# huangjh-pub/di-fusion

Measured on AMD Instinct MI355X. Metric: frames/s integrate+decode+mesh, 640x480 synthetic stream, higher is better.
Workload: dtype f32

## Files before the change

### di_fusion_amd/_lib.py

```python
from __future__ import annotations

import ctypes
import os
from ctypes import POINTER, Structure, c_float, c_int32, c_int64, c_uint8, c_void_p
from pathlib import Path

PKG = Path(__file__).resolve().parent
LIB_PATH = Path(os.environ["DIF_LIB"]) if os.environ.get("DIF_LIB") else PKG / "libdifusion.so"

C_N_OCCUPIED, C_OVERFLOW, C_ALLOC_NEW, C_M, C_C, C_ITEMS, C_K, C_B, C_VH, C_T, C_QUERY_M, C_N_KEPT, C_CACHE_T, C_CACHE_KEPT, C_EXPORT_N, C_WORK, C_CACHE_DEAD, C_CACHE_LIVE, C_OPT_ROWS, C_OPT_VOXELS, C_HALO_L, C_HALO_R, C_HALO_TICKET, C_DEFERRED = range(24)
C_STAMP = 31
SYNC_FUSED, SYNC_FRONT_DONE, SYNC_WORDS = 0, 32, 64
FC_COUNT = 32
C_COUNT = 32
PROF_NAMES = ["encode", "decode_lattice", "decode_points", "mc_count", "mc_emit", "halo_export", "halo_merge"]
PROF_COUNT = 8
LATENT_DIM = 29

ERRORS = {-1: "DIF_EINVAL (bad argument)", -2: "DIF_ELAUNCH (HIP launch/runtime failure)", -3: "DIF_ENOSPACE (workspace too small)"}


class DifMap(Structure):
    _fields_ = [("nx", c_int32), ("ny", c_int32), ("nz", c_int32),
                ("bound_min", c_float * 3), ("voxel_size", c_float),
# ... 65 lines not shown
    "dif_compute_normal_weight": (c_int32, [c_void_p, c_void_p, c_int32, c_int32, c_void_p]),
    "dif_filter_depth": (c_int32, [c_void_p, c_void_p, c_int32, c_int32, c_void_p]),
    "dif_depth_frontend": (c_int32, [c_void_p, c_int32, c_int32, c_float, c_float, c_float, c_float, c_int32, c_void_p, c_void_p, c_void_p,
                                     c_void_p, c_void_p, c_void_p]),
    "dif_point_box_filter": (c_int32, [c_void_p, c_void_p, c_int64, c_float, c_void_p, c_void_p, c_void_p, c_void_p, c_int64, c_void_p,
                                       c_void_p, c_void_p, c_void_p]),
    "dif_cloud_workspace_bytes": (c_int64, [c_int64]),
    "dif_knn": (c_int32, [c_void_p, c_int64, c_int32, c_int32, c_float, c_void_p, c_void_p, c_void_p, c_int64, c_void_p]),
    "dif_remove_radius_outlier": (c_int32, [c_void_p, c_int64, c_int32, c_int32, c_float, c_void_p, c_void_p, c_int64, c_void_p]),
    "dif_estimate_normals": (c_int32, [c_void_p, c_int64, c_int32, c_int32, c_float, POINTER(c_float), c_void_p, c_void_p, c_int64,
                                       c_void_p]),
    "dif_groupby_sum": (c_int32, [c_void_p, c_void_p, c_int64, c_int32, c_void_p, c_void_p, c_int64, c_void_p]),
    "dif_integrate_workspace_bytes": (c_int64, [c_int64]),
    "dif_integrate": (c_int32, [POINTER(DifMap), POINTER(DifWeights), c_void_p, c_void_p, c_int64, c_void_p, c_void_p,
                                c_int64, c_void_p]),
    "dif_integrate_frame": (c_int32, [POINTER(DifMap), POINTER(DifWeights), c_void_p, c_int32, c_int32, c_float, c_float, c_float, c_float,
                                      c_void_p, c_void_p, c_void_p, c_void_p, c_int64, c_void_p]),
    "dif_optimize_workspace_bytes": (c_int64, [c_int64, c_int64]),
    "dif_optimize_latents": (c_int32, [POINTER(DifMap), POINTER(DifWeights), c_void_p, c_void_p, c_int64, c_void_p, c_void_p, c_int32, c_float,
                                       c_float, c_void_p, c_void_p, c_int64, c_void_p]),
    "dif_extract": (c_int32, [POINTER(DifMap), POINTER(DifWeights), POINTER(DifExtractBuffers), c_int32, c_int32, c_float,
                              c_int32, c_int32, c_void_p]),
    "dif_integrate_frames": (c_int32, [POINTER(DifStreamFrame), c_int32, POINTER(DifWeights), c_int32, c_int32, c_float, c_float, c_float, c_float,
                                       c_void_p]),
    "dif_extract_streams": (c_int32, [POINTER(DifStreamFrame), c_int32, POINTER(DifWeights), c_int32, c_float, c_int32, c_void_p]),
    "dif_export_pending": (c_int32, [POINTER(DifMap), c_void_p]),
    "dif_mesh_cache_export": (c_int32, [POINTER(DifExtractBuffers), c_int64, c_int64, c_void_p, c_void_p, c_void_p, c_void_p]),
    "dif_mesh_cache_export_dma": (c_int32, [POINTER(DifExtractBuffers), c_int64, c_int64, c_void_p, c_void_p, c_void_p, c_void_p]),
    "dif_mesh_cache_compact": (c_int32, [POINTER(DifMap), POINTER(DifExtractBuffers), c_void_p, c_void_p, c_void_p, c_int64, c_void_p, c_void_p]),
    "dif_mesh_cache_reindex": (c_int32, [POINTER(DifMap), POINTER(DifExtractBuffers), c_int64, c_void_p]),
    "dif_marching_cubes": (c_int32, [c_void_p, c_int32, c_int32, c_int32, c_void_p, c_int64, c_void_p, c_int64, c_void_p,
                                     c_void_p, c_int32, c_float, c_int64, c_void_p, c_void_p, c_void_p, c_void_p,
                                     c_void_p, c_void_p, c_void_p, c_void_p]),
    "dif_decode_rows": (c_int32, [POINTER(DifWeights), c_void_p, c_int64, c_void_p, c_void_p, c_void_p]),
    "dif_encode_rows": (c_int32, [POINTER(DifWeights), c_void_p, c_int64, c_void_p, c_void_p]),
    "dif_query_sdf": (c_int32, [POINTER(DifMap), POINTER(DifWeights), c_void_p, c_int64, c_void_p, c_void_p, c_void_p,
                                c_void_p, c_void_p, c_void_p, c_void_p]),
    "dif_query_select": (c_int32, [POINTER(DifMap), c_void_p, c_int64, c_void_p, c_void_p, c_void_p, c_void_p, c_int32, c_void_p]),
    "dif_query_decode": (c_int32, [POINTER(DifMap), POINTER(DifWeights), c_void_p, c_int64, c_void_p, c_void_p, c_void_p, c_void_p, c_void_p]),
    "dif_query_grad_scatter": (c_int32, [c_void_p, c_void_p, c_void_p, c_int64, c_void_p, c_void_p]),
    "dif_query_grad_gather": (c_int32, [c_void_p, c_void_p, c_void_p, c_int64, c_void_p, c_void_p]),
    "dif_export_records": (c_int32, [POINTER(DifMap), c_void_p, c_int64, c_int32, c_int32, c_int32, c_void_p, c_void_p]),
    "dif_merge_records": (c_int32, [POINTER(DifMap), c_void_p, c_int64, c_int32, c_void_p, c_void_p]),
    "dif_export_halo": (c_int32, [POINTER(DifMap), c_void_p, c_int64, c_int32, c_int32, c_void_p, c_void_p]),
    "dif_merge_halo": (c_int32, [POINTER(DifMap), c_void_p, c_int64, c_void_p, c_void_p]),
    "dif_export_halo_delta": (c_int32, [POINTER(DifMap), c_void_p, c_void_p, c_int64, c_void_p, c_void_p]),
    "dif_halo_lists_reset": (c_int32, [POINTER(DifMap), c_void_p, c_void_p, c_void_p, c_void_p]),
    "dif_merge_halo2": (c_int32, [POINTER(DifMap), c_void_p, c_int64, c_void_p, c_int64, c_void_p, c_void_p, c_void_p]),
    "dif_profile_enable": (c_int32, [c_int32]),
    "dif_profile_read": (c_int32, [POINTER(ctypes.c_double), POINTER(c_int64), c_int32]),
    "dif_profile_dump": (c_int64, [POINTER(c_int32), POINTER(c_float), c_int64, c_int32]),
    "dif_read_counters": (c_int32, [POINTER(DifMap), POINTER(c_int32), c_void_p]),
    "dif_test_mc_grid_cap": (c_int32, [c_int32]),
    "dif_test_sdma_mode": (c_int32, [c_int32]),
    "dif_sdma_info": (c_int32, [POINTER(c_int32)]),
    "dif_test_handoff": (c_int32, [c_int32, c_int32, c_int32, c_int32, POINTER(c_int64)]),
    "dif_queues_independent": (c_int32, [c_void_p, c_void_p]),
    "dif_mesh_cache_export_sdma": (c_int32, [POINTER(DifExtractBuffers), c_int64, c_int64, c_void_p, c_void_p, c_void_p]),
    "dif_sdf_hg_workspace_bytes": (c_int64, [c_int64]),
    "dif_sdf_hg": (c_int32, [POINTER(DifMap), POINTER(DifWeights), c_void_p, c_int64, POINTER(DifSdfHg), c_void_p, c_int64, c_void_p, c_void_p,
                             c_int64, c_void_p]),
    "dif_gradient_xy": (c_int32, [c_void_p, c_int32, c_int32, c_void_p, c_void_p]),
    "dif_photo_pyramid": (c_int32, [c_void_p, c_void_p, c_int32, c_int32, POINTER(DifPhotoPyramid), c_void_p]),
    "dif_rgb_odometry": (c_int32, [c_void_p, c_void_p, c_void_p, c_void_p, c_void_p, c_int32, c_int32, POINTER(DifRgbHg), c_void_p, c_void_p,
                                   c_void_p]),
    "dif_rgb_hg_workspace_bytes": (c_int64, []),
    "dif_rgb_hg": (c_int32, [c_void_p, c_void_p, c_void_p, c_void_p, c_void_p, c_int32, c_int32, POINTER(DifRgbHg), c_void_p, c_int64, c_void_p,
                             c_void_p, c_int64, c_void_p]),
}

_lib = None


def load() -> ctypes.CDLL:
    global _lib
    if _lib is None:
        import torch
        if not LIB_PATH.exists():
            raise RuntimeError(f"{LIB_PATH} is missing: build it with `python -c 'import __graft_entry__ as g; g.build()'` "
                               "(hipcc, gfx950). di_fusion_amd has no CPU fallback.")
        if not os.environ.get("DIF_LIB"):
            from . import _build
            have, want = _build.lib_build_id(), _build.source_hash()
            if have != want:
                try:
                    _build.build(force=True, verbose=False, shared=True)
                except Exception as e:
                    raise RuntimeError(f"{LIB_PATH} was built from other sources (build id {have}, tree {want}) and rebuilding it failed: {e!r}")
        lib = ctypes.CDLL(str(LIB_PATH))
        for name, (res, args) in SIGNATURES.items():
            fn = getattr(lib, name)
            fn.restype = res
            fn.argtypes = args
        _lib = lib
    return _lib


def spin_until(words, index: int, value: int, what: str, timeout_s: float = 30.0):
    import time
    if words[index] == value:
        return
    t0 = time.perf_counter()
    n = 0
    while words[index] != value:
        n += 1
        if (n & 0x3FFF) == 0 and time.perf_counter() - t0 > timeout_s:
# ... 29 lines not shown
```

### di_fusion_amd/csrc/difusion.hip

```cpp
#include <cstdlib>
#include <cstdio>
#include <cstring>
#include <mutex>
#include <atomic>
#include <chrono>
#include <vector>
#include <hip/hip_runtime.h>
#include <hsa/hsa.h>
#include <hsa/hsa_ext_amd.h>
#include <dlfcn.h>

#include "common.hip.h"
#include "mlp.hip.h"
#include "mc_tables.inc"

using namespace dif;

namespace {

constexpr int L = DIF_LATENT_DIM;

__device__ __constant__ int c_mc_edge_table[256];
__device__ __constant__ unsigned long long c_mc_tri_packed[256];
bool g_tables_uploaded[64] = {};
// ... 859 lines not shown
    a.max_triangles = buf->cache_capacity; a.new_limit = buf->max_triangles; a.base_ptr = C + DIF_C_CACHE_KEPT;
    a.triangles = buf->cache_tri; a.tri_id = buf->cache_id; a.tri_std = buf->cache_std; a.tri_alive = buf->cache_alive;
    a.scale = scale_vertices ? 1 : 0; a.vs = map->voxel_size; a.bx = map->bound_min[0]; a.by = map->bound_min[1]; a.bz = map->bound_min[2];
    a.log_counters = C;
    a.grid_tot = map->grid_tot;
    if (2 * (e.r + 1) * (e.r + 1) * (e.r + 1) <= e.R3) {
        a.corner_cache = reinterpret_cast<float*>(buf->refine_list);
        a.corner_stride = e.R3;
    }
    return a;
}

static bool defer_export_of(const dif_map_t* map, const dif_extract_buffers_t* buf) {
    return buf->defer_export && map->pending_export && buf->out_tri && buf->out_id && buf->out_std;
}

static void mc_onepass_args(McArgs& a, const dif_map_t* map, const dif_extract_buffers_t* buf, bool defer) {
    a.tri_start = map->tri_start; a.tri_n = map->tri_n; a.tri_count = buf->tri_count; a.tri_offset = nullptr;
    if (!defer && buf->out_tri && buf->out_id && buf->out_std) {
        a.out_tri = buf->out_tri; a.out_id = buf->out_id; a.out_std = buf->out_std; a.out_capacity = buf->out_capacity;
    }
}

static FinishArgs finish_args_of(const dif_map_t* map, const dif_extract_buffers_t* buf, bool fused_scan, bool onepass, bool exported, bool defer) {
    int32_t* const super_sum = buf->chunk_sum ? buf->chunk_sum + (buf->max_voxels + 255) / 256 : nullptr;
    const bool ov = overlapped(map);
    return FinishArgs{buf->occ_slot, map->vbm, map->counters, buf->max_triangles, buf->cache_capacity, buf->cache_tri, buf->cache_id, buf->cache_std,
                      ExtractOut{buf->counters_out, buf->out_tri, buf->out_id, buf->out_std, buf->out_capacity, (exported || defer) ? 1 : 0,
                                 defer ? (dif_pending_export_t*)map->pending_export : nullptr, buf->stamp, defer ? buf->export_notify : nullptr},
                      (fused_scan && !onepass) ? buf->chunk_sum : nullptr, super_sum, map->dirty_tot, (int)((map->capacity + DIF_BLOCK - 1) / DIF_BLOCK),
                      onepass ? buf->mc_status : nullptr, onepass ? buf->mc_status + (buf->max_voxels + 3) / 4 : nullptr,
                      ov ? map->frame_counters : nullptr};
}

static int voxel_decode_attributes() {
    static bool attr_set[64] = {};
    int dev = 0; (void)hipGetDevice(&dev);
    if (dev < 64 && !attr_set[dev]) {
        const int fp32_bytes = (int)(((size_t)((DEC_LDS_FLOATS + 3) & ~3) + 4 * VD_WAVE_LDS_FLOATS) * 4);
        const int x6_bytes = (int)((size_t)X6_LDS_BYTES + 4 * VD_WAVE_LDS_FLOATS * 4);
        if (hipFuncSetAttribute((const void*)k_decode_voxels<false>, hipFuncAttributeMaxDynamicSharedMemorySize, fp32_bytes) != hipSuccess) return DIF_ELAUNCH;
        if (hipFuncSetAttribute((const void*)k_decode_voxels<true>, hipFuncAttributeMaxDynamicSharedMemorySize, x6_bytes) != hipSuccess) return DIF_ELAUNCH;
        if (hipFuncSetAttribute((const void*)k_decode_refine_x6, hipFuncAttributeMaxDynamicSharedMemorySize, (int)X6_LDS_BYTES) != hipSuccess) return DIF_ELAUNCH;
        if (hipFuncSetAttribute((const void*)k_decode_voxels_batch<true>, hipFuncAttributeMaxDynamicSharedMemorySize, x6_bytes) != hipSuccess) return DIF_ELAUNCH;
        if (hipFuncSetAttribute((const void*)k_decode_refine_x6_batch, hipFuncAttributeMaxDynamicSharedMemorySize, (int)X6_LDS_BYTES) != hipSuccess) return DIF_ELAUNCH;
        attr_set[dev] = true;
    }
    return DIF_OK;
}

static std::atomic<int> g_mc_grid_cap{0};
int dif_test_mc_grid_cap(int32_t n) { return g_mc_grid_cap.exchange(n > 0 ? n : 0); }

static int mc_onepass_setup(const McArgs& a, size_t& lds_bytes, int& grid1, int64_t max_voxels) {
    if (upload_tables() != DIF_OK) return DIF_ELAUNCH;
    const int r = a.R / 2, nc = (r + 1) * (r + 1) * (r + 1);
    lds_bytes = (size_t)(DIF_BLOCK / 64) * MC_ONEPASS_WAVE_LDS_FLOATS(nc) * sizeof(float);
    if (lds_bytes > 128 * 1024) return DIF_EINVAL;
    static bool attr_set1[64] = {};
    int dev = 0; (void)hipGetDevice(&dev);
    if (dev < 64 && !attr_set1[dev]) {
        if (hipFuncSetAttribute((const void*)k_marching_cubes_onepass<0>, hipFuncAttributeMaxDynamicSharedMemorySize, 128 * 1024) != hipSuccess) return DIF_ELAUNCH;
        if (hipFuncSetAttribute((const void*)k_marching_cubes_onepass<4>, hipFuncAttributeMaxDynamicSharedMemorySize, 128 * 1024) != hipSuccess) return DIF_ELAUNCH;
        if (hipFuncSetAttribute((const void*)k_marching_cubes_onepass_batch<0>, hipFuncAttributeMaxDynamicSharedMemorySize, 128 * 1024) != hipSuccess) return DIF_ELAUNCH;
        if (hipFuncSetAttribute((const void*)k_marching_cubes_onepass_batch<4>, hipFuncAttributeMaxDynamicSharedMemorySize, 128 * 1024) != hipSuccess) return DIF_ELAUNCH;
        attr_set1[dev] = true;
    }
    const int64_t need = (max_voxels + 3) / 4;
    int per_cu = (int)((160 * 1024) / (lds_bytes + 1024));
    per_cu = per_cu < 1 ? 1 : per_cu > MC_WAVES_PER_SIMD ? MC_WAVES_PER_SIMD : per_cu;
    grid1 = per_cu * num_cus();
    if (need < grid1) grid1 = (int)(need < 1 ? 1 : need);
    { const int n = g_mc_grid_cap.load(std::memory_order_relaxed); if (n > 0 && n < grid1) grid1 = n; }
    return DIF_OK;
}

static int extract_mesh_part(const dif_map_t* map, const dif_extract_buffers_t* buf, const ExtractGeo& e, float max_std, int32_t no_cache,
                             int32_t scale_vertices, hipStream_t s);

static int extract_impl(const dif_map_t* map, const dif_weights_t* w, const dif_extract_buffers_t* buf, int32_t resolution, int32_t fast,
                        float max_std, int32_t no_cache, int32_t scale_vertices, void* stream_) {
    if (!map || !w || !buf || resolution < 1 || resolution > 8 || buf->max_voxels <= 0) return DIF_EINVAL;
    const int* n_slots = map->counters + DIF_C_N_OCCUPIED;
    if (!map->grid_tot) return DIF_EINVAL;
    const GridMarks bits = grid_marks_of(map);
    if (buf->cache_capacity <= 0 || buf->cache_capacity >= ((int64_t)1 << 31) || !buf->cache_tri || !buf->cache_id || !buf->cache_std || !buf->cache_alive)
        return DIF_EINVAL;
    if (!map->tri_start || !map->tri_n) return DIF_EINVAL;
    hipStream_t s = (hipStream_t)stream_;
    const int64_t grid = (int64_t)map->nx * map->ny * map->nz;
    Geo g = geo_of(map);
    int* C = map->counters;
    const bool ov = overlapped(map);
    if (ov && (!overlap_ok(map) || no_cache || defer_export_of(map, buf) || s != (hipStream_t)map->fuse_stream)) return DIF_EINVAL;
    const ExtractGeo e = extract_geo(resolution);
    const int r = e.r, R = e.R, l = e.l, R3 = e.R3;
    if (buf->max_voxels * (int64_t)R3 >= ((int64_t)1 << 31)) return DIF_EINVAL;
    const double sample_a = e.sample_a, sample_b = e.sample_b;

    {
        const DirtySet ds = dirty_set_of(map, buf, no_cache);
        const bool tiled = ds.tiled;
        if (tiled) {
            hipLaunchKernelGGL(k_mark_halo_dirty, dim3(grid_for(map->capacity, DIF_BLOCK, 256)), dim3(DIF_BLOCK), 0, s, g, map->ignore_count_th, map->dirty,
                               (const int64_t*)map->latent_vecs_pos, (const int64_t*)map->indexer, (const float*)map->voxel_obs_count, bits,
                               n_slots, ds.own_lin_lo, ds.own_lin_hi);
            DIF_CHECK_LAUNCH();
        }
        {
            DirtyFunctor f{ds};
            if (map->dirty_tot && !no_cache && !tiled && map->capacity > 4096 && map->capacity % DIF_BLOCK == 0) {
                hipLaunchKernelGGL(k_dirty_scan, dim3((int)(map->capacity / DIF_BLOCK)), dim3(DIF_BLOCK), 0, s, ds, n_slots, (const int*)map->dirty_tot,
                                   ov ? map->sync_words + DIF_SYNC_FUSED : nullptr, (int)map->frame_seq);
                DIF_CHECK_LAUNCH();
            } else if (ov) {
                return DIF_EINVAL;
            } else if (map->dirty_tot && !no_cache && !tiled) {
                if (launch_counted_scan_bounded(f, n_slots, map->capacity, map->dirty_tot, s) != DIF_OK) return DIF_ELAUNCH;
            } else if (launch_scan(f, n_slots, 0, map->capacity, buf->block_tmp, s) != DIF_OK) return DIF_ELAUNCH;
        }
    }
    {
        OccFunctor f{map->grid_bits, map->indexer, buf->occ_slot, map->vbm, C, buf->max_voxels};
        if (launch_counted_scan(f, (int)((grid + 31) / 32), map->grid_tot, s) != DIF_OK) return DIF_ELAUNCH;
    }
    int rc;
    if (fast && l * l * l <= VD_MAX_L3 && R * R <= VD_MAX_R2) {
        if (!w->dec_packed || w->dec_packed_floats != DEC_FLOATS) return DIF_EINVAL;
        const bool fold = w->dec_fold_packed && w->dec_fold_packed_floats == DECF_FLOATS && buf->fold_table;
        const VoxelDecodeArgs V = voxel_decode_args_of(map, w, buf, e, fold);
        const bool x6 = fold && w->dec_x6_packed && w->dec_x6_packed_bytes == X6_BYTES;
        const size_t lds_bytes = x6 ? (size_t)X6_LDS_BYTES + 4 * VD_WAVE_LDS_FLOATS * 4
                                    : ((size_t)((DEC_LDS_FLOATS + 3) & ~3) + 4 * VD_WAVE_LDS_FLOATS) * 4;
        if (voxel_decode_attributes() != DIF_OK) return DIF_ELAUNCH;
        int64_t blocks = (buf->max_voxels + 3) / 4;
        if (blocks > num_cus()) blocks = num_cus();
        {
            ProfScope prof(DIF_PROF_DECODE_LATTICE, s);
            if (x6) hipLaunchKernelGGL(k_decode_voxels<true>, dim3((int)blocks), dim3(512), lds_bytes, s, V, (const float*)w->dec_x6_packed);
            else hipLaunchKernelGGL(k_decode_voxels<false>, dim3((int)blocks), dim3(512), lds_bytes, s, V, w->dec_packed);
        }
        DIF_CHECK_LAUNCH();
        const DecodeArgs Rf = refine_args_of(map, buf, e, fold);
        if (x6) {
            int64_t rblocks = (buf->max_voxels * (int64_t)(R3 / 32) + 7) / 8;
            if (rblocks < 1) rblocks = 1;
            if (rblocks > num_cus()) rblocks = num_cus();
            ProfScope prof(DIF_PROF_DECODE_POINTS, s);
            hipLaunchKernelGGL(k_decode_refine_x6, dim3((int)rblocks), dim3(512), (size_t)X6_LDS_BYTES, s, Rf, (const float*)w->dec_x6_packed);
            DIF_CHECK_LAUNCH();
            rc = DIF_OK;
        } else {
            rc = launch_decode(Rf, w, buf->max_voxels * (int64_t)(R3 / 32), s);
        }
        if (rc != DIF_OK) return rc;
    } else if (fast) {
        DecodeArgs A = {};
        A.mode = 0; A.n_ptr = C + DIF_C_B; A.occ_slot = buf->occ_slot; A.latent = map->latent_vecs;
        A.lat.res = l; A.lat.a = (float)sample_a;
        A.lat.vsize = (l > 1) ? (float)((sample_b - sample_a) / (l - 1)) : 0.0f;
        A.out_sdf = buf->low_sdf; A.out_std = buf->low_std; A.sign = 1.0f;
        rc = launch_decode(A, w, buf->max_voxels * ((l * l * l + 31) / 32), s);
        if (rc != DIF_OK) return rc;
        hipLaunchKernelGGL(k_upsample_mark, dim3(grid_for(buf->max_voxels * (int64_t)(R * R), DIF_BLOCK, 4096)), dim3(DIF_BLOCK), 0, s,
                           (const float*)buf->low_sdf, (const float*)buf->low_std, l, R, buf->cube_sdf, buf->cube_std, buf->refine_list, C);
        DIF_CHECK_LAUNCH();
        const DecodeArgs Rf = refine_args_of(map, buf, e, false);
        rc = launch_decode(Rf, w, buf->max_voxels * (int64_t)(R3 / 32), s);
        if (rc != DIF_OK) return rc;
    } else {
        DecodeArgs A = {};
        A.mode = 0; A.n_ptr = C + DIF_C_B; A.occ_slot = buf->occ_slot; A.latent = map->latent_vecs;
        A.lat.res = R; A.lat.a = (float)sample_a; A.lat.vsize = (float)((sample_b - sample_a) / (R - 1));
        A.out_sdf = buf->cube_sdf; A.out_std = buf->cube_std; A.sign = -1.0f;
        rc = launch_decode(A, w, buf->max_voxels * (int64_t)((R3 + 31) / 32), s);
        if (rc != DIF_OK) return rc;
    }
    return extract_mesh_part(map, buf, e, max_std, no_cache, scale_vertices, s);
}

static int extract_mesh_part(const dif_map_t* map, const dif_extract_buffers_t* buf, const ExtractGeo& e, float max_std, int32_t no_cache,
                             int32_t scale_vertices, hipStream_t s) {
    int* C = map->counters;
    const int r = e.r;
    int rc;
    McArgs a = mc_args_of(map, buf, e, max_std, scale_vertices);
    if (no_cache) {
        if (hipMemsetAsync(C + DIF_C_CACHE_T, 0, sizeof(int), s) != hipSuccess) return DIF_ELAUNCH;
        if (hipMemsetAsync(C + DIF_C_CACHE_DEAD, 0, sizeof(int), s) != hipSuccess) return DIF_ELAUNCH;
// ... 35 lines not shown
        ts.new_limit = buf->max_triangles; ts.capacity = buf->cache_capacity;
        rc = mc_count_and_scan(a, buf->max_voxels, buf->tri_count, buf->tri_offset, buf->block_tmp, C, ts, s);
        if (rc != DIF_OK) return rc;
        rc = mc_emit(a, buf->max_voxels, buf->tri_count, buf->tri_offset, s);
        if (rc != DIF_OK) return rc;
    }
    hipLaunchKernelGGL(k_extract_finish, dim3(grid_for(buf->max_voxels, DIF_BLOCK, 256)), dim3(DIF_BLOCK), 0, s,
                       finish_args_of(map, buf, fused_scan, onepass, onepass && a.out_tri, defer));
    DIF_CHECK_LAUNCH();
    return DIF_OK;
}

int dif_extract_streams(const dif_stream_frame_t* st, int32_t S, const dif_weights_t* w, int32_t resolution, float max_std, int32_t scale_vertices,
                        void* stream_) {
    if (!batch_maps_ok(st, S) || !w || resolution < 1 || resolution > 4) return DIF_EINVAL;
    const ExtractGeo e = extract_geo(resolution);
    if (e.l * e.l * e.l > VD_MAX_L3 || e.R * e.R > VD_MAX_R2 || e.r * e.r * e.r > 64) return DIF_EINVAL;
    if (!w->dec_packed || w->dec_packed_floats != DEC_FLOATS || !w->dec_fold_packed || w->dec_fold_packed_floats != DECF_FLOATS || !w->dec_x6_packed ||
        w->dec_x6_packed_bytes != X6_BYTES)
        return DIF_EINVAL;
    const dif_map_t* m0 = st[0].map;
    if (m0->capacity <= 4096 || m0->capacity % DIF_BLOCK != 0) return DIF_EINVAL;
    const int64_t grid = (int64_t)m0->nx * m0->ny * m0->nz;
    static thread_local Batch<DirtyScanArgs> dirty; static thread_local ScanBatch<OccFunctor> occ; static thread_local Batch<VoxelDecodeArgs> vd;
    static thread_local Batch<DecodeArgs> rf; static thread_local Batch<McStream> mc; static thread_local Batch<FinishArgs> fin;
    for (int j = 0; j < S; ++j) {
        const dif_map_t* map = st[j].map;
        const dif_extract_buffers_t* buf = st[j].buf;
        if (!buf || buf->max_voxels <= 0 || buf->max_voxels != st[0].buf->max_voxels || buf->max_voxels * (int64_t)e.R3 >= ((int64_t)1 << 31)) return DIF_EINVAL;
        if (buf->cache_capacity <= 0 || buf->cache_capacity >= ((int64_t)1 << 31) || !buf->cache_tri || !buf->cache_id || !buf->cache_std || !buf->cache_alive)
            return DIF_EINVAL;
        if (!map->tri_start || !map->tri_n || !buf->fold_table || !buf->chunk_sum || !buf->mc_status || buf->max_voxels > ((int64_t)1 << 24)) return DIF_EINVAL;
        dirty.s[j] = DirtyScanArgs{dirty_set_of(map, buf, 0), map->counters + DIF_C_N_OCCUPIED, map->dirty_tot};
        occ.f[j] = OccFunctor{map->grid_bits, map->indexer, buf->occ_slot, map->vbm, map->counters, buf->max_voxels};
        occ.tot[j] = map->grid_tot;
        vd.s[j] = voxel_decode_args_of(map, w, buf, e, true);
        rf.s[j] = refine_args_of(map, buf, e, true);
        const bool defer = defer_export_of(map, buf);
        McArgs a = mc_args_of(map, buf, e, max_std, scale_vertices);
        mc_onepass_args(a, map, buf, defer);
        mc.s[j] = McStream{a, buf->mc_status, buf->mc_status + (buf->max_voxels + 3) / 4};
        fin.s[j] = finish_args_of(map, buf, true, true, a.out_tri != nullptr, defer);
    }
    for (int j = S; j < DIF_MAX_STREAMS; ++j) {
        dirty.s[j] = dirty.s[0]; occ.f[j] = occ.f[0]; occ.tot[j] = occ.tot[0]; vd.s[j] = vd.s[0]; rf.s[j] = rf.s[0]; mc.s[j] = mc.s[0]; fin.s[j] = fin.s[0];
    }
    hipStream_t s = (hipStream_t)stream_;
    const int64_t max_voxels = st[0].buf->max_voxels;
    hipLaunchKernelGGL(k_dirty_scan_batch, dim3((int)(m0->capacity / DIF_BLOCK), S), dim3(DIF_BLOCK), 0, s, dirty);
    DIF_CHECK_LAUNCH();
    if (launch_counted_scan_batch(occ, S, (int)((grid + 31) / 32), s) != DIF_OK) return DIF_ELAUNCH;
    if (voxel_decode_attributes() != DIF_OK) return DIF_ELAUNCH;
    {
        int64_t blocks = (max_voxels * S + 3) / 4;
        if (blocks > num_cus()) blocks = num_cus();
        ProfScope prof(DIF_PROF_DECODE_LATTICE, s);
        hipLaunchKernelGGL(k_decode_voxels_batch<true>, dim3((int)blocks), dim3(512), (size_t)X6_LDS_BYTES + 4 * VD_WAVE_LDS_FLOATS * 4, s, vd, (int)S,
                           (const float*)w->dec_x6_packed);
        DIF_CHECK_LAUNCH();
    }
    {
        int64_t rblocks = (max_voxels * S * (int64_t)(e.R3 / 32) + 7) / 8;
        if (rblocks < 1) rblocks = 1;
        if (rblocks > num_cus()) rblocks = num_cus();
        ProfScope prof(DIF_PROF_DECODE_POINTS, s);
        hipLaunchKernelGGL(k_decode_refine_x6_batch, dim3((int)rblocks), dim3(512), (size_t)X6_LDS_BYTES, s, rf, (int)S, (const float*)w->dec_x6_packed);
        DIF_CHECK_LAUNCH();
    }
    {
        size_t lds_bytes; int grid1;
        const int rc = mc_onepass_setup(mc.s[0].a, lds_bytes, grid1, max_voxels);
        if (rc != DIF_OK) return rc;
        ProfScope prof(DIF_PROF_MC_COUNT, s);
        if (e.r == 4) hipLaunchKernelGGL(k_marching_cubes_onepass_batch<4>, dim3(grid1, S), dim3(DIF_BLOCK), lds_bytes, s, mc);
        else hipLaunchKernelGGL(k_marching_cubes_onepass_batch<0>, dim3(grid1, S), dim3(DIF_BLOCK), lds_bytes, s, mc);
        DIF_CHECK_LAUNCH();
    }
    hipLaunchKernelGGL(k_extract_finish_batch, dim3(grid_for(max_voxels, DIF_BLOCK, 256), S), dim3(DIF_BLOCK), 0, s, fin);
    DIF_CHECK_LAUNCH();
    return DIF_OK;
}

#ifdef DIF_TRACE
int dif_trace_read(unsigned long long* out, int64_t n) {
    return hipMemcpyFromSymbol(out, HIP_SYMBOL(g_vd_trace), (size_t)n * 8) == hipSuccess ? DIF_OK : DIF_ELAUNCH;
}
int dif_trace_read_encode(unsigned long long* out, int64_t n) {
    return hipMemcpyFromSymbol(out, HIP_SYMBOL(g_en_trace), (size_t)n * 8) == hipSuccess ? DIF_OK : DIF_ELAUNCH;
}
#endif

int dif_extract(const dif_map_t* map, const dif_weights_t* w, const dif_extract_buffers_t* buf, int32_t resolution, int32_t fast,
                float max_std, int32_t no_cache, int32_t scale_vertices, void* stream_) {
    return extract_impl(map, w, buf, resolution, fast, max_std, no_cache, scale_vertices, stream_);
}

int dif_export_pending(const dif_map_t* map, void* stream) {
    if (!map) return DIF_EINVAL;
    if (!map->pending_export) return DIF_OK;
    hipStream_t s = (hipStream_t)stream;
    hipLaunchKernelGGL(k_export_pending, dim3(DIF_EXPORT_WGS), dim3(DIF_BLOCK), 0, s, (dif_pending_export_t*)map->pending_export);
    DIF_CHECK_LAUNCH();
    if (hipMemsetAsync(map->pending_export, 0, sizeof(int32_t), s) != hipSuccess) return DIF_ELAUNCH;
    return DIF_OK;
}

int dif_mesh_cache_export(const dif_extract_buffers_t* buf, int64_t lo, int64_t n, float* out_tri, int64_t* out_id, float* out_std, void* stream) {
    if (!buf || lo < 0 || n < 0 || lo + n > buf->cache_capacity || (n > 0 && (!out_tri || !out_id || !out_std))) return DIF_EINVAL;
// ... 619 lines not shown
```

### di_fusion_amd/csrc/kernels_extract.hip.h

```cpp
#pragma once

__device__ __forceinline__ void mark_confident_nbhd(const Geo& g, int lin, float ignore_th, const int64_t* __restrict__ indexer,
                                                    const float* __restrict__ obs, const GridMarks& marks) {
    const uint32_t* bits = marks.bits;
    int ix, iy, iz;
    unlinearize(g, lin, ix, iy, iz);
    int cand[7];
    cand[0] = lin;
    cand[1] = linearize(g, clampi(ix - 1, 0, g.nx - 1), iy, iz);
    cand[2] = linearize(g, clampi(ix + 1, 0, g.nx - 1), iy, iz);
    cand[3] = linearize(g, ix, clampi(iy - 1, 0, g.ny - 1), iz);
    cand[4] = linearize(g, ix, clampi(iy + 1, 0, g.ny - 1), iz);
    cand[5] = linearize(g, ix, iy, clampi(iz - 1, 0, g.nz - 1));
    cand[6] = linearize(g, ix, iy, clampi(iz + 1, 0, g.nz - 1));
    int64_t slot[7];
#pragma unroll
    for (int c = 0; c < 7; ++c) slot[c] = indexer[cand[c]];
    float w[7];
#pragma unroll
    for (int c = 0; c < 7; ++c) w[c] = slot[c] >= 0 ? obs[slot[c]] : ignore_th;
    uint32_t word[7];
#pragma unroll
    for (int c = 0; c < 7; ++c) word[c] = (w[c] > ignore_th) ? bits[cand[c] >> 5] : 0xFFFFFFFFu;
    uint32_t prev[7];
// ... 498 lines not shown
        unsigned sel = 0;
        int64_t e0 = 0;
        if (row < n_rows) {
            const int b = (int)(row / R2), jxy = (int)(row - (int64_t)b * R2);
            const int jx = jxy / R, jy = jxy % R;
            int x0, x1, y0, y1; float wx0, wx1, wy0, wy1;
            tri_axis(jx, l, scale, x0, x1, wx0, wx1);
            tri_axis(jy, l, scale, y0, y1, wy0, wy1);
            const float* ls = low_sdf + (int64_t)b * l3;
            const float* ld = low_std + (int64_t)b * l3;
            e0 = (int64_t)b * R3 + (int64_t)jxy * R;
            NO_PACKED_F32
            for (int jz = 0; jz < R; ++jz) {
                int z0, z1; float wz0, wz1;
                tri_axis(jz, l, scale, z0, z1, wz0, wz1);
                float sv = tri_sample(ls, l, x0, x1, y0, y1, z0, z1, wx0, wx1, wy0, wy1, wz0, wz1);
                float dv = tri_sample(ld, l, x0, x1, y0, y1, z0, z1, wx0, wx1, wy0, wy1, wz0, wz1);
                cube_sdf[e0 + jz] = -sv;
                cube_std[e0 + jz] = dv;
                if (fabsf(sv) < 0.05f) sel |= 1u << jz;
            }
        }
        int total;
        int ex = block_excl_scan(__popc(sel), smem, total);
        if (total > 0) {
            if (threadIdx.x == 0) s_base = atomicAdd(counters + DIF_C_VH, total);
            __syncthreads();
            int o = s_base + ex;
            while (sel) {
                int jz = __ffs((int)sel) - 1;
                sel &= sel - 1;
                refine_list[o++] = (int32_t)(e0 + jz);
            }
        }
        __syncthreads();
    }
}

struct VoxelDecodeArgs {
    const int32_t* occ_slot;
    const float* latent;
    Lattice low;
    int R;
    float* cube_sdf;
    float* cube_std;
    int32_t* refine_list;
    int* counters;
    const float* fold_w;
    float* fold_table;
};

#define VD_MAX_L3 64
#define VD_MAX_R2 64
#define VD_WAVE_LDS_FLOATS (2 * VD_MAX_L3 + 2 * 256)

#ifdef DIF_TRACE
__device__ unsigned long long g_vd_trace[2048 * 8];
#define VD_STAMP(slot) do { if (lane_id() == 0) g_vd_trace[((threadIdx.x >> 6) * gridDim.x + blockIdx.x) * 8 + (slot)] = wall_clock64(); } while (0)
#else
#define VD_STAMP(slot) do { } while (0)
#endif

template <bool X6, int NS>
__device__ __forceinline__ void decode_voxels_body(const BatchN<VoxelDecodeArgs, NS>& AB, int S, const float* __restrict__ wblob) {
    extern __shared__ __attribute__((aligned(16))) float lds[];
    VD_STAMP(0);
    constexpr int LDS_W = X6 ? X6_LDS_BYTES / 4 : ((DEC_LDS_FLOATS + 3) & ~3);
#if defined(DIF_VD_CUT) && DIF_VD_CUT == 0
    return;
#endif
    stage_weights(lds, wblob, X6 ? X6_LDS_BYTES / 4 : DEC_LDS_FLOATS);
    VD_STAMP(1);
#if defined(DIF_VD_CUT) && DIF_VD_CUT == 1
    return;
#endif
    const __amdgpu_buffer_rsrc_t wfwd = make_rsrc(wblob, X6 ? X6_BYTES / 4 : DEC_FLOATS);
    const int lane = lane_id(), half = lane >> 5, col = lane & 31, wid = threadIdx.x >> 6;
    const int pair = wid >> 1, tsel = wid & 1;
    float* w_low_sdf = lds + LDS_W + pair * VD_WAVE_LDS_FLOATS;
    float* w_low_std = w_low_sdf + VD_MAX_L3;
    float* w_fold = w_low_std + VD_MAX_L3 + tsel * 256;
    const Lattice low = AB.s[0].low;
    const float* const fold_w = AB.s[0].fold_w;
    const int l = low.res, R = AB.s[0].R, l3 = l * l * l, R2 = R * R, R3 = R2 * R;
    const float scale = (float)(l - 1) / (float)(R - 1);
    int pre[NS + 1];
    pre[0] = 0;
#pragma unroll
    for (int j = 0; j < NS; ++j) pre[j + 1] = pre[j] + ((j < S) ? AB.s[j].counters[DIF_C_B] : 0);
    const int B = pre[NS];
    const int pairs_per_block = (int)(blockDim.x >> 7), n_pairs = (int)gridDim.x * pairs_per_block;
    const int first = __builtin_amdgcn_readfirstlane(pair * (int)gridDim.x + (int)blockIdx.x);
    __shared__ int s_tot[8], s_map[8], s_base[NS];
    const int rounds = (B + n_pairs - 1) / n_pairs;
    for (int round = 0; round < rounds; ++round) {
        const int bg = first + round * n_pairs;
        int sm = 0, b = bg;
#pragma unroll
        for (int j = 1; j < NS; ++j)
            if (bg >= pre[j]) { sm = j; b = bg - pre[j]; }
        const VoxelDecodeArgs& A = AB.s[sm];
        unsigned sel = 0;
        const int jz0 = tsel * (R >> 1), jz1 = jz0 + (R >> 1);
        const int64_t e0 = (int64_t)b * R3 + (int64_t)lane * R;
        if (bg < B && tsel * 32 < l3) {
            const float* lat_row = A.latent + (int64_t)A.occ_slot[b] * L;
            const int s = tsel * 32 + col;
            const float px = low.coord(s / (l * l)), py = low.coord((s / l) % l), pz = low.coord(s % l);
            float sdf = 0.0f, sd = 0.0f;
            if (X6 || fold_w) {
                if constexpr (X6) decoder_fold_consts_x6(lds, fold_w, lat_row, w_fold, lane);
                else decoder_fold_consts(lds, fold_w, lat_row, w_fold, lane);
                __builtin_amdgcn_wave_barrier();
                __builtin_amdgcn_s_waitcnt(0xc07f);
                if (tsel == 0) {
                    float* rec = A.fold_table + (int64_t)b * 256;
                    for (int p = lane; p < 256; p += 64) rec[p] = w_fold[p];
                }
                VD_STAMP(6);
#if defined(DIF_VD_CUT) && DIF_VD_CUT == 2
                sdf = w_fold[lane]; sd = w_fold[lane + 64];
#else
                if constexpr (X6) decoder_tile_folded_x6(lds, wfwd, FoldInitLds{w_fold}, px, py, pz, lane, sdf, sd);
                else decoder_tile_folded(lds, wfwd, FoldInitLds{w_fold}, px, py, pz, lane, sdf, sd);
#endif
            } else if constexpr (!X6) {
                f16v xin;
#pragma unroll
                for (int t = 0; t < 16; ++t) {
                    const int k = 2 * t + half;
                    xin[t] = (k < L) ? lat_row[k] : 0.0f;
                }
                if (half) { xin[14] = px; xin[15] = pz; } else { xin[15] = py; }
                decoder_tile(lds, wfwd, xin, lane, sdf, sd);
            }
            if (s < l3) {
                if (half == 0) w_low_sdf[s] = sdf;
                else w_low_std[s] = sd;
            }
        }
        __syncthreads();
        VD_STAMP(2);
        if (bg < B && lane < R2) {
            const int jx = lane / R, jy = lane % R;
            int x0, x1, y0, y1; float wx0, wx1, wy0, wy1;
            tri_axis(jx, l, scale, x0, x1, wx0, wx1);
            tri_axis(jy, l, scale, y0, y1, wy0, wy1);
            float* const cube_sdf = A.cube_sdf;
            float* const cube_std = A.cube_std;
            for (int jz = jz0; jz < jz1; ++jz) {
                int z0, z1; float wz0, wz1;
                tri_axis(jz, l, scale, z0, z1, wz0, wz1);
                float sv = tri_sample(w_low_sdf, l, x0, x1, y0, y1, z0, z1, wx0, wx1, wy0, wy1, wz0, wz1);
                float dv = tri_sample(w_low_std, l, x0, x1, y0, y1, z0, z1, wx0, wx1, wy0, wy1, wz0, wz1);
                cube_sdf[e0 + jz] = -sv;
                cube_std[e0 + jz] = dv;
                if (fabsf(sv) < 0.05f) sel |= 1u << jz;
            }
        }
        VD_STAMP(3);
        const int c = __popc(sel);
        const int incl = wave_incl_scan(c);
        const int total = __shfl(incl, 63);
        if (lane == 0) { s_tot[wid] = total; if (NS > 1) s_map[wid] = sm; }
        __syncthreads();
        if (NS == 1) {
            if (threadIdx.x == 0) {
                int sum = 0;
                for (int w = 0; w < (int)(blockDim.x >> 6); ++w) sum += s_tot[w];
                s_base[0] = sum ? atomicAdd(A.counters + DIF_C_VH, sum) : 0;
            }
        } else if ((int)threadIdx.x < S) {
            const int j = (int)threadIdx.x;
            int sum = 0;
            for (int w = 0; w < (int)(blockDim.x >> 6); ++w) sum += (s_map[w] == j) ? s_tot[w] : 0;
            s_base[j] = sum ? atomicAdd(AB.s[j].counters + DIF_C_VH, sum) : 0;
        }
        __syncthreads();
        if (total > 0) {
            int o = s_base[NS == 1 ? 0 : sm] + incl - c;
            for (int w = 0; w < wid; ++w) o += (NS == 1 || s_map[w] == sm) ? s_tot[w] : 0;
            int32_t* const refine_list = A.refine_list;
            while (sel) {
                const int jz = __ffs((int)sel) - 1;
                sel &= sel - 1;
                refine_list[o++] = (int32_t)(e0 + jz);
            }
        }
        __syncthreads();
        VD_STAMP(4);
    }
    VD_STAMP(5);
}

template <bool X6>
__global__ void __launch_bounds__(512, X6 ? 1 : 2) k_decode_voxels(VoxelDecodeArgs A, const float* __restrict__ wblob) {
    const BatchN<VoxelDecodeArgs, 1> B{{A}};
    decode_voxels_body<X6, 1>(B, 1, wblob);
}
template <bool X6>
__global__ void __launch_bounds__(512, X6 ? 1 : 2) k_decode_voxels_batch(Batch<VoxelDecodeArgs> B, int S, const float* __restrict__ wblob) {
    decode_voxels_body<X6, DIF_MAX_STREAMS>(B, S, wblob);
}
```

### include/difusion.h

```cpp
#ifndef DIFUSION_H
#define DIFUSION_H

#include <stdint.h>

#ifdef __cplusplus
extern "C" {
#endif

#define DIF_VERSION 100
#define DIF_LATENT_DIM 29

#define DIF_MAX_STREAMS 8

#define DIF_OK 0
#define DIF_EINVAL (-1)
#define DIF_ELAUNCH (-2)
#define DIF_ENOSPACE (-3)

enum {
    DIF_C_N_OCCUPIED = 0,
    DIF_C_OVERFLOW = 1,
    DIF_C_ALLOC_NEW = 2,
    DIF_C_M = 3,
    DIF_C_C = 4,
// ... 220 lines not shown
int64_t dif_sdf_hg_workspace_bytes(int64_t N);
int dif_sdf_hg(const dif_map_t* map, const dif_weights_t* w, const float* obs_xyz, int64_t N, const dif_sdf_hg_t* args, void* ws, int64_t ws_bytes,
               double* out, double* out_host, int64_t seq, void* stream);

int dif_gradient_xy(const float* intensity, int32_t H, int32_t W, float* out, void* stream);
typedef struct dif_photo_pyramid_t {
    float* intensity[3];
    float* depth[3];
    float* gradient[3];
} dif_photo_pyramid_t;
int dif_photo_pyramid(const float* rgb, const float* depth, int32_t H, int32_t W, const dif_photo_pyramid_t* out, void* stream);
typedef struct dif_rgb_hg_t {
    float krkinv[9];
    float kt[3];
    float intr[4];
    float min_grad_scale;
    float max_depth_delta;
    float weight;
    int32_t robust_kernel;
    float robust_k;
    int32_t no_grad;
} dif_rgb_hg_t;
int dif_rgb_odometry(const float* prev_I, const float* prev_D, const float* cur_I, const float* cur_D, const float* cur_G, int32_t H, int32_t W,
                     const dif_rgb_hg_t* args, float* f_out, float* J_out, void* stream);
int64_t dif_rgb_hg_workspace_bytes(void);
int dif_rgb_hg(const float* prev_I, const float* prev_D, const float* cur_I, const float* cur_D, const float* cur_G, int32_t H, int32_t W,
               const dif_rgb_hg_t* args, void* ws, int64_t ws_bytes, double* out, double* out_host, int64_t seq, void* stream);

int dif_export_records(const dif_map_t* map, int32_t* records, int64_t max_records, int32_t x_lo, int32_t x_hi, int32_t raw,
                       int32_t* scratch, void* stream);
int dif_merge_records(const dif_map_t* map, const int32_t* records, int64_t n, int32_t assign, int32_t* scratch, void* stream);

int dif_export_halo(const dif_map_t* map, int32_t* message, int64_t max_records, int32_t x_lo, int32_t x_hi, int32_t* scratch, void* stream);
int dif_merge_halo(const dif_map_t* map, const int32_t* message, int64_t max_records, int32_t* scratch, void* stream);
int dif_export_halo_delta(const dif_map_t* map, int32_t* msg_left, int32_t* msg_right, int64_t max_records, int32_t* note, void* stream);
int dif_halo_lists_reset(const dif_map_t* map, int32_t* header_left, int32_t* header_right, int32_t* note, void* stream);
int dif_merge_halo2(const dif_map_t* map, const int32_t* msg_a, int64_t max_a, const int32_t* msg_b, int64_t max_b, int32_t* scratch,
                    int32_t* note, void* stream);

enum { DIF_PROF_ENCODE = 0, DIF_PROF_DECODE_LATTICE = 1, DIF_PROF_DECODE_POINTS = 2, DIF_PROF_MC_COUNT = 3, DIF_PROF_MC_EMIT = 4,
       DIF_PROF_HALO_EXPORT = 5 , DIF_PROF_HALO_MERGE = 6 ,
       DIF_PROF_COUNT = 8 };
int dif_profile_enable(int32_t on);
int dif_profile_read(double* ms , int64_t* launches , int32_t reset);
int64_t dif_profile_dump(int32_t* which , float* ms , int64_t capacity, int32_t reset);

int dif_read_counters(const dif_map_t* map, int32_t* host_out , void* stream);

int dif_queues_independent(void* stream_a, void* stream_b);

int dif_mesh_cache_export_sdma(const dif_extract_buffers_t* buf, int64_t lo, int64_t n, float* out_tri, int64_t* out_id, float* out_std);

int dif_test_mc_grid_cap(int32_t n);
int dif_test_sdma_mode(int32_t mode);
int dif_test_handoff(int32_t mode, int32_t groups, int32_t iters, int32_t flags, int64_t* out);
int dif_sdma_info(int32_t* out);

#ifdef __cplusplus
}
#endif
#endif
```

Measured before the change: 9481.

## Replace block barriers in voxel decode with pairwise LDS flags and deferred list writes

```diff
diff --git a/di_fusion_amd/_lib.py b/di_fusion_amd/_lib.py
--- a/di_fusion_amd/_lib.py
+++ b/di_fusion_amd/_lib.py
@@ -141,6 +141,7 @@
     "dif_profile_dump": (c_int64, [POINTER(c_int32), POINTER(c_float), c_int64, c_int32]),
     "dif_read_counters": (c_int32, [POINTER(DifMap), POINTER(c_int32), c_void_p]),
     "dif_test_mc_grid_cap": (c_int32, [c_int32]),
+    "dif_test_decode_grid_cap": (c_int32, [c_int32]),
     "dif_test_sdma_mode": (c_int32, [c_int32]),
     "dif_sdma_info": (c_int32, [POINTER(c_int32)]),
     "dif_test_handoff": (c_int32, [c_int32, c_int32, c_int32, c_int32, POINTER(c_int64)]),
diff --git a/di_fusion_amd/csrc/difusion.hip b/di_fusion_amd/csrc/difusion.hip
--- a/di_fusion_amd/csrc/difusion.hip
+++ b/di_fusion_amd/csrc/difusion.hip
@@ -935,6 +935,16 @@
 static std::atomic<int> g_mc_grid_cap{0};
 int dif_test_mc_grid_cap(int32_t n) { return g_mc_grid_cap.exchange(n > 0 ? n : 0); }
 
+static std::atomic<int> g_decode_grid_cap{0};
+int dif_test_decode_grid_cap(int32_t n) { return g_decode_grid_cap.exchange(n > 0 ? n : 0); }
+static int64_t voxel_decode_blocks(int64_t voxels) {
+    int64_t blocks = (voxels + 3) / 4;
+    if (blocks > num_cus()) blocks = num_cus();
+    const int n = g_decode_grid_cap.load(std::memory_order_relaxed);
+    if (n > 0 && n < blocks) blocks = n;
+    return blocks;
+}
+
 static int mc_onepass_setup(const McArgs& a, size_t& lds_bytes, int& grid1, int64_t max_voxels) {
     if (upload_tables() != DIF_OK) return DIF_ELAUNCH;
     const int r = a.R / 2, nc = (r + 1) * (r + 1) * (r + 1);
@@ -1016,8 +1026,7 @@
         const size_t lds_bytes = x6 ? (size_t)X6_LDS_BYTES + 4 * VD_WAVE_LDS_FLOATS * 4
                                     : ((size_t)((DEC_LDS_FLOATS + 3) & ~3) + 4 * VD_WAVE_LDS_FLOATS) * 4;
         if (voxel_decode_attributes() != DIF_OK) return DIF_ELAUNCH;
-        int64_t blocks = (buf->max_voxels + 3) / 4;
-        if (blocks > num_cus()) blocks = num_cus();
+        const int64_t blocks = voxel_decode_blocks(buf->max_voxels);
         {
             ProfScope prof(DIF_PROF_DECODE_LATTICE, s);
             if (x6) hipLaunchKernelGGL(k_decode_voxels<true>, dim3((int)blocks), dim3(512), lds_bytes, s, V, (const float*)w->dec_x6_packed);
@@ -1159,8 +1168,7 @@
     if (launch_counted_scan_batch(occ, S, (int)((grid + 31) / 32), s) != DIF_OK) return DIF_ELAUNCH;
     if (voxel_decode_attributes() != DIF_OK) return DIF_ELAUNCH;
     {
-        int64_t blocks = (max_voxels * S + 3) / 4;
-        if (blocks > num_cus()) blocks = num_cus();
+        const int64_t blocks = voxel_decode_blocks(max_voxels * S);
         ProfScope prof(DIF_PROF_DECODE_LATTICE, s);
         hipLaunchKernelGGL(k_decode_voxels_batch<true>, dim3((int)blocks), dim3(512), (size_t)X6_LDS_BYTES + 4 * VD_WAVE_LDS_FLOATS * 4, s, vd, (int)S,
                            (const float*)w->dec_x6_packed);
diff --git a/di_fusion_amd/csrc/kernels_extract.hip.h b/di_fusion_amd/csrc/kernels_extract.hip.h
--- a/di_fusion_amd/csrc/kernels_extract.hip.h
+++ b/di_fusion_amd/csrc/kernels_extract.hip.h
@@ -574,7 +574,8 @@
 
 #define VD_MAX_L3 64
 #define VD_MAX_R2 64
-#define VD_WAVE_LDS_FLOATS (2 * VD_MAX_L3 + 2 * 256)
+#define VD_WAVE_LDS_FLOATS (4 * VD_MAX_L3 + 2 * 256)
+#define VD_SPIN_LIMIT (1 << 20)
 
 #ifdef DIF_TRACE
 __device__ unsigned long long g_vd_trace[2048 * 8];
@@ -582,6 +583,15 @@
 #else
 #define VD_STAMP(slot) do { } while (0)
 #endif
+
+__device__ __forceinline__ void vd_wait_ge(int* word, int value, int* counters) {
+    int spins = 0;
+    while (__builtin_amdgcn_readfirstlane(__hip_atomic_load(word, __ATOMIC_RELAXED, __HIP_MEMORY_SCOPE_WORKGROUP)) < value) {
+        if (++spins > VD_SPIN_LIMIT) { if (lane_id() == 0) counters[DIF_C_OVERFLOW] = 9; break; }
+        __builtin_amdgcn_s_sleep(1);
+    }
+    __builtin_amdgcn_fence(__ATOMIC_ACQUIRE, "workgroup");
+}
 
 template <bool X6, int NS>
 __device__ __forceinline__ void decode_voxels_body(const BatchN<VoxelDecodeArgs, NS>& AB, int S, const float* __restrict__ wblob) {
@@ -591,6 +601,11 @@
 #if defined(DIF_VD_CUT) && DIF_VD_CUT == 0
     return;
 #endif
+    __shared__ int s_pair[4];
+    __shared__ int s_tot[2][NS], s_base[2][NS], s_arrive[2], s_ready[2];
+    if (threadIdx.x < 4) s_pair[threadIdx.x] = 0;
+    if (threadIdx.x < 2 * NS) (&s_tot[0][0])[threadIdx.x] = 0;
+    if (threadIdx.x < 2) { s_arrive[threadIdx.x] = 0; s_ready[threadIdx.x] = 0; }
     stage_weights(lds, wblob, X6 ? X6_LDS_BYTES / 4 : DEC_LDS_FLOATS);
     VD_STAMP(1);
 #if defined(DIF_VD_CUT) && DIF_VD_CUT == 1
@@ -599,9 +614,8 @@
     const __amdgpu_buffer_rsrc_t wfwd = make_rsrc(wblob, X6 ? X6_BYTES / 4 : DEC_FLOATS);
     const int lane = lane_id(), half = lane >> 5, col = lane & 31, wid = threadIdx.x >> 6;
     const int pair = wid >> 1, tsel = wid & 1;
-    float* w_low_sdf = lds + LDS_W + pair * VD_WAVE_LDS_FLOATS;
-    float* w_low_std = w_low_sdf + VD_MAX_L3;
-    float* w_fold = w_low_std + VD_MAX_L3 + tsel * 256;
+    float* const w_rec = lds + LDS_W + pair * VD_WAVE_LDS_FLOATS;
+    float* w_fold = w_rec + 4 * VD_MAX_L3 + tsel * 256;
     const Lattice low = AB.s[0].low;
     const float* const fold_w = AB.s[0].fold_w;
     const int l = low.res, R = AB.s[0].R, l3 = l * l * l, R2 = R * R, R3 = R2 * R;
@@ -611,17 +625,37 @@
 #pragma unroll
     for (int j = 0; j < NS; ++j) pre[j + 1] = pre[j] + ((j < S) ? AB.s[j].counters[DIF_C_B] : 0);
     const int B = pre[NS];
-    const int pairs_per_block = (int)(blockDim.x >> 7), n_pairs = (int)gridDim.x * pairs_per_block;
+    const int pairs_per_block = (int)(blockDim.x >> 7), n_pairs = (int)gridDim.x * pairs_per_block, n_waves = (int)(blockDim.x >> 6);
     const int first = __builtin_amdgcn_readfirstlane(pair * (int)gridDim.x + (int)blockIdx.x);
-    __shared__ int s_tot[8], s_map[8], s_base[NS];
     const int rounds = (B + n_pairs - 1) / n_pairs;
+    unsigned p_sel = 0;
+    int p_b = 0, p_sm = 0, p_off = 0, p_total = 0;
+    auto list_round = [&](int r) {
+        const int par = r & 1;
+        vd_wait_ge(&s_ready[par], r + 1, AB.s[0].counters);
+        if (p_total > 0) {
+            const int c = __popc(p_sel);
+            int o = s_base[par][NS == 1 ? 0 : p_sm] + p_off + wave_incl_scan(c) - c;
+            const int64_t e0 = (int64_t)p_b * R3 + (int64_t)lane * R;
+            int32_t* const refine_list = AB.s[p_sm].refine_list;
+            while (p_sel) {
+                const int jz = __ffs((int)p_sel) - 1;
+                p_sel &= p_sel - 1;
+                refine_list[o++] = (int32_t)(e0 + jz);
+            }
+        }
+        VD_STAMP(4);
+    };
     for (int round = 0; round < rounds; ++round) {
+        const int par = round & 1;
         const int bg = first + round * n_pairs;
         int sm = 0, b = bg;
 #pragma unroll
         for (int j = 1; j < NS; ++j)
             if (bg >= pre[j]) { sm = j; b = bg - pre[j]; }
         const VoxelDecodeArgs& A = AB.s[sm];
+        float* const w_low_sdf = w_rec + par * 2 * VD_MAX_L3;
+        float* const w_low_std = w_low_sdf + VD_MAX_L3;
         unsigned sel = 0;
         const int jz0 = tsel * (R >> 1), jz1 = jz0 + (R >> 1);
         const int64_t e0 = (int64_t)b * R3 + (int64_t)lane * R;
@@ -661,57 +695,62 @@
                 else w_low_std[s] = sd;
             }
         }
-        __syncthreads();
+        __builtin_amdgcn_s_waitcnt(0xc07f);
+        __builtin_amdgcn_fence(__ATOMIC_RELEASE, "workgroup");
+        if (lane == 0) __hip_atomic_fetch_add(&s_pair[pair], 1, __ATOMIC_RELAXED, __HIP_MEMORY_SCOPE_WORKGROUP);
+        if (round > 0) list_round(round - 1);
+        vd_wait_ge(&s_pair[pair], 2 * (round + 1), AB.s[0].counters);
         VD_STAMP(2);
-        if (bg < B && lane < R2) {
-            const int jx = lane / R, jy = lane % R;
-            int x0, x1, y0, y1; float wx0, wx1, wy0, wy1;
-            tri_axis(jx, l, scale, x0, x1, wx0, wx1);
-            tri_axis(jy, l, scale, y0, y1, wy0, wy1);
+        const bool row = bg < B && lane < R2;
+        int x0 = 0, x1 = 0, y0 = 0, y1 = 0; float wx0 = 0.0f, wx1 = 0.0f, wy0 = 0.0f, wy1 = 0.0f;
+        if (row) {
+            tri_axis(lane / R, l, scale, x0, x1, wx0, wx1);
+            tri_axis(lane % R, l, scale, y0, y1, wy0, wy1);
             float* const cube_sdf = A.cube_sdf;
-            float* const cube_std = A.cube_std;
+            NO_PACKED_F32
             for (int jz = jz0; jz < jz1; ++jz) {
                 int z0, z1; float wz0, wz1;
                 tri_axis(jz, l, scale, z0, z1, wz0, wz1);
                 float sv = tri_sample(w_low_sdf, l, x0, x1, y0, y1, z0, z1, wx0, wx1, wy0, wy1, wz0, wz1);
-                float dv = tri_sample(w_low_std, l, x0, x1, y0, y1, z0, z1, wx0, wx1, wy0, wy1, wz0, wz1);
                 cube_sdf[e0 + jz] = -sv;
-                cube_std[e0 + jz] = dv;
                 if (fabsf(sv) < 0.05f) sel |= 1u << jz;
             }
         }
+        const int total = __shfl(wave_incl_scan(__popc(sel)), 63);
+        int off = 0, before = 0;
+        if (lane == 0) {
+            if (total > 0) off = __hip_atomic_fetch_add(&s_tot[par][NS == 1 ? 0 : sm], total, __ATOMIC_RELAXED, __HIP_MEMORY_SCOPE_WORKGROUP);
+            before = __hip_atomic_fetch_add(&s_arrive[par], 1, __ATOMIC_ACQ_REL, __HIP_MEMORY_SCOPE_WORKGROUP);
+        }
+        const bool last = __builtin_amdgcn_readfirstlane(before) == n_waves - 1;
+        p_sel = sel; p_b = b; p_sm = sm; p_total = total;
+        p_off = __builtin_amdgcn_readfirstlane(off);
+        int g_base = 0;
+        if (last && lane < NS) {
+            const int sum = s_tot[par][lane];
+            int vh = DIF_C_VH;
+            asm volatile("" : "+v"(vh));
+            if (sum) g_base = atomicAdd(AB.s[NS == 1 ? 0 : lane].counters + vh, sum);
+        }
+        if (row) {
+            float* const cube_std = A.cube_std;
+            NO_PACKED_F32
+            for (int jz = jz0; jz < jz1; ++jz) {
+                int z0, z1; float wz0, wz1;
+                tri_axis(jz, l, scale, z0, z1, wz0, wz1);
+                cube_std[e0 + jz] = tri_sample(w_low_std, l, x0, x1, y0, y1, z0, z1, wx0, wx1, wy0, wy1, wz0, wz1);
+            }
+        }
         VD_STAMP(3);
-        const int c = __popc(sel);
-        const int incl = wave_incl_scan(c);
-        const int total = __shfl(incl, 63);
-        if (lane == 0) { s_tot[wid] = total; if (NS > 1) s_map[wid] = sm; }
-        __syncthreads();
-        if (NS == 1) {
-            if (threadIdx.x == 0) {
-                int sum = 0;
-                for (int w = 0; w < (int)(blockDim.x >> 6); ++w) sum += s_tot[w];
-                s_base[0] = sum ? atomicAdd(A.counters + DIF_C_VH, sum) : 0;
-            }
-        } else if ((int)threadIdx.x < S) {
-            const int j = (int)threadIdx.x;
-            int sum = 0;
-            for (int w = 0; w < (int)(blockDim.x >> 6); ++w) sum += (s_map[w] == j) ? s_tot[w] : 0;
-            s_base[j] = sum ? atomicAdd(AB.s[j].counters + DIF_C_VH, sum) : 0;
-        }
-        __syncthreads();
-        if (total > 0) {
-            int o = s_base[NS == 1 ? 0 : sm] + incl - c;
-            for (int w = 0; w < wid; ++w) o += (NS == 1 || s_map[w] == sm) ? s_tot[w] : 0;
-            int32_t* const refine_list = A.refine_list;
-            while (sel) {
-                const int jz = __ffs((int)sel) - 1;
-                sel &= sel - 1;
-                refine_list[o++] = (int32_t)(e0 + jz);
-            }
-        }
-        __syncthreads();
-        VD_STAMP(4);
-    }
+        if (last) {
+            if (lane < NS) { s_base[par][lane] = g_base; s_tot[par][lane] = 0; }
+            if (lane == 0) s_arrive[par] = 0;
+            __builtin_amdgcn_s_waitcnt(0xc07f);
+            __builtin_amdgcn_fence(__ATOMIC_RELEASE, "workgroup");
+            if (lane == 0) __hip_atomic_store(&s_ready[par], round + 1, __ATOMIC_RELAXED, __HIP_MEMORY_SCOPE_WORKGROUP);
+        }
+    }
+    if (rounds > 0) list_round(rounds - 1);
     VD_STAMP(5);
 }
 
diff --git a/include/difusion.h b/include/difusion.h
--- a/include/difusion.h
+++ b/include/difusion.h
@@ -296,6 +296,7 @@
 int dif_mesh_cache_export_sdma(const dif_extract_buffers_t* buf, int64_t lo, int64_t n, float* out_tri, int64_t* out_id, float* out_std);
 
 int dif_test_mc_grid_cap(int32_t n);
+int dif_test_decode_grid_cap(int32_t n);
 int dif_test_sdma_mode(int32_t mode);
 int dif_test_handoff(int32_t mode, int32_t groups, int32_t iters, int32_t flags, int64_t* out);
 int dif_sdma_info(int32_t* out);
```

New measurement: 9722, median of 4. 1.03x the previous value.
